# goalheart/ionic-mpnn

Hardware: AMD Instinct MI355X
Metric: molecule-graph pairs/sec (fwd), batch 4096 per MI355X (higher is better)
Workload: dtype f32 (bf16x9 emulation)

## Files before the change

ionic_mpnn_amd/csrc/api.hip:

```cpp
#include <cstring>
#include <vector>

#include <cstddef>

#include "common.h"
#include "encoder_layout.h"

namespace impnn {

char* error_buffer() {
  static thread_local char buf[512] = {0};
  return buf;
}

int fail(int code, const char* fmt, ...) {
  va_list ap;
  va_start(ap, fmt);
  vsnprintf(error_buffer(), 512, fmt, ap);
  va_end(ap);
  return code;
}

namespace {
struct Profiler {
// ... 313 lines not shown
                "indices or row offsets: split the batch", B, N, E, D);
  *bytes = encoder_fused_workspace_bytes(mode, n_ions, B, N, E, D, S, Vb, encoder_workgroups(n_ions, B, workgroups, N, E, mode));
  return IMPNN_OK;
}

int impnn_encoder_plan_layout(int32_t n_ions, int32_t B, int32_t N, int32_t E, int32_t D, int32_t K, int32_t S,
                              int32_t Vb, int32_t mode, int32_t workgroups, int64_t out[8]) {
  REQUIRE(out, "null pointer");
  size_t total = 0;
  if (int rc = impnn_encoder_workspace_bytes(n_ions, B, N, E, D, K, S, Vb, mode, workgroups, &total)) return rc;
  if (D != enc::kD)
    return fail(IMPNN_E_UNSUPPORTED, "encoder_plan_layout: atom_dim %d has no chunk plan (atom_dim 32 only)", D);
  const bool typed = mode >= 2;
  const int nwg = encoder_workgroups(n_ions, B, workgroups, N, E, mode);
  const enc::Ws w = enc::ws_layout(n_ions, B, N, E, S, Vb, nwg, typed, mode == 3);
  out[0] = w.nwg;
  out[1] = w.max_sub;
  out[2] = (int64_t)w.rows_off;
  out[3] = (int64_t)w.vr_off;
  out[4] = (int64_t)w.nsub_off;
  out[5] = (int64_t)w.desc_off;
  out[6] = typed ? enc::tecap_of(E) : 0;
  out[7] = enc::plan_vmin(n_ions, B, enc::vr_max_of(N, E, typed), w.nwg);
  return IMPNN_OK;
}

int impnn_encoder_plan_records(int32_t n_ions, int32_t B, int32_t N, int32_t E, int32_t D, int32_t K, int32_t S,
                               int32_t Vb, int32_t mode, int32_t workgroups, int64_t out[5]) {
  REQUIRE(out, "null pointer");
  size_t total = 0;
  if (int rc = impnn_encoder_workspace_bytes(n_ions, B, N, E, D, K, S, Vb, mode, workgroups, &total)) return rc;
  if (D != enc::kD)
    return fail(IMPNN_E_UNSUPPORTED, "encoder_plan_records: atom_dim %d has no chunk plan (atom_dim 32 only)", D);
  if (mode < 2)
    return fail(IMPNN_E_UNSUPPORTED, "encoder_plan_records: mode %d has pull-form records (typed modes only)", mode);
  const int nwg = encoder_workgroups(n_ions, B, workgroups, N, E, mode);
  const enc::Ws w = enc::ws_layout(n_ions, B, N, E, S, Vb, nwg, true, mode == 3);
  out[0] = (int64_t)w.rec_off;
  out[1] = w.rec_bytes;
  out[2] = enc::kTRecGrp;
  out[3] = enc::trec_runs_off(Vb, enc::tecap_of(E));
  out[4] = enc::kTRecNrun;
  return IMPNN_OK;
}

static int encoder_common(const char* fn, int32_t n_ions, const int32_t* const* atom_ids,
// ... 1632 lines not shown
```

ionic_mpnn_amd/csrc/common.h:

```cpp
#pragma once

#include <hip/hip_runtime.h>

#include <cstdarg>
#include <cstdint>
#include <cstdio>

#include "../../include/impnn.h"

namespace impnn {

char* error_buffer();
int fail(int code, const char* fmt, ...);

inline hipStream_t as_stream(impnn_stream_t s) { return reinterpret_cast<hipStream_t>(s); }

inline int check_launch(const char* what) {
  hipError_t e = hipGetLastError();
  if (e != hipSuccess) return fail(IMPNN_E_LAUNCH, "%s: %s", what, hipGetErrorString(e));
  return IMPNN_OK;
}

inline bool aligned16(const void* p) { return (reinterpret_cast<uintptr_t>(p) & 15u) == 0; }

// ... 422 lines not shown

void* debug_stamp_buffer(size_t* bytes);

struct EncoderArgs {
  int n_ions;
  const int32_t* atom_ids[2];
  const int32_t* bond_ids[2];
  const int32_t* conn[2];
  const float* weights[2];
  const void* prepared[2];
  int mode;
  int phases;
  int nwg;
  float* pooled[2];
  const float* atom_table;
  const float* bond_table;
  int Va, Vb, B, N, E, D, K, S;
  float ln_eps;
  void* workspace;
  size_t workspace_bytes;
};
bool encoder_fused_supported(int mode, int N, int E, int D, int K, int S, int Vb);
int encoder_workgroups(int n_ions, int B, int requested, int N, int E, int mode);
size_t encoder_fused_workspace_bytes(int mode, int n_ions, int B, int N, int E, int D, int S, int Vb, int nwg);
int launch_encoder_fused(const EncoderArgs& a, hipStream_t s);
int launch_encoder_phase(const EncoderArgs& a, hipStream_t s, bool plan_phase);
size_t encoder_prepared_bytes(int mode, int D, int S, int Vb);
int launch_encoder_prepare(const float* weights, const float* bond_table, int D, int K, int S, int Vb, int mode,
                           void* prepared, hipStream_t s);
size_t encoder_prepared_bytes_atoms(int mode, int D, int S, int Va, int Vb);
int launch_encoder_prepare_atoms(const float* weights, const float* bond_table, const float* atom_table, int Va, int D,
                                 int K, int S, int Vb, int mode, void* prepared, hipStream_t s);
size_t encoder_prepared_bytes_gates(int mode, int D, int S, int Va, int Vb);
int launch_encoder_prepare_gates(const float* weights, const float* bond_table, const float* atom_table, int Va, int D,
                                 int K, int S, int Vb, int mode, void* prepared, hipStream_t s);
int ensure_lds_limit(const void* kern, int slot);
int device_compute_units();
inline int gu_wide_tile_rows(int64_t rows) { return rows < 8192 ? 16 : 64; }
bool encoder_wide_supported(int N, int E, int D, int K, int S, int Vb);
size_t encoder_wide_workspace_bytes(int n_ions, int B, int N, int E, int D, int S, int Vb, bool x3);
bool encoder_wide_batch_covered(int n_ions, int B, int N, int E, int D, int Vb);
size_t encoder_wide_prepared_bytes(int D, int S, int Vb, bool x3);
int launch_encoder_wide_prepare(const float* weights, const float* bond_table, int D, int K, int S, int Vb, bool x3,
                                void* prepared, hipStream_t s);
int launch_encoder_wide(const EncoderArgs& a, hipStream_t s);

// ... 2 lines not shown
```

ionic_mpnn_amd/csrc/encoder_fused.hip:

```cpp
#include <atomic>
#include <cstdlib>

#include "encoder_device.h"
#include "encoder_layout.h"

namespace impnn {
namespace enc {

namespace {

struct H8 {
  half8 hi, lo;
};
__device__ __forceinline__ H8 split8(const float* v) {
  typedef __fp16 h2_t __attribute__((ext_vector_type(2)));
  union U {
    h2_t h;
    unsigned u;
  };
  union {
    half8 v8;
    unsigned u[4];
  } hi, lo;
#pragma unroll
// ... 452 lines not shown
  if (e != hipSuccess) return fail(IMPNN_E_LAUNCH, "encoder: cannot raise LDS limit: %s", hipGetErrorString(e));
  done[slot].fetch_or(bit, std::memory_order_release);
  return IMPNN_OK;
}

int encoder_workgroups(int n_ions, int B, int requested, int N, int E, int mode) {
  int cus = device_compute_units();
  int want = requested;
  if (want <= 0) {
    static const int env_want = [] {
      const char* e = getenv("IMPNN_ENCODER_WORKGROUPS");
      return e ? atoi(e) : 0;
    }();
    want = env_want;
  }
  if (want > 0) cus = want < 16 ? 16 : (want > cus ? cus : want);
  int f = 1;
  while ((int64_t)2 * n_ions * B / ((int64_t)cus * f) + 64 > enc::kShareCap ||
         enc::ws_layout(n_ions, B, N, E, 1, 1, cus * f, mode >= 2, mode == 3).max_sub > enc::kMaxHops)
    ++f;
  return cus * f;
}

size_t encoder_fused_workspace_bytes(int mode, int n_ions, int B, int N, int E, int D, int S, int Vb, int nwg) {
  if (D != enc::kD) return encoder_wide_workspace_bytes(n_ions, B, N, E, D, S, Vb, mode == 3);
  return enc::ws_layout(n_ions, B, N, E, S, Vb, nwg, mode >= 2, mode == 3).total;
}

size_t encoder_prepared_bytes(int mode, int D, int S, int Vb) {
  if (D != enc::kD) return encoder_wide_prepared_bytes(D, S, Vb, mode == 3);
  if (mode >= 2) return encoder_typed_prepared_bytes(S, Vb, mode == 3);
  return (size_t)(S > 0 ? S : 1) * enc::kImgSlot * sizeof(float);
}

int launch_encoder_prepare(const float* weights, const float* bond_table, int D, int K, int S, int Vb, int mode,
                           void* prepared, hipStream_t s) {
  if (S <= 0) return IMPNN_OK;
  if (D != enc::kD) return launch_encoder_wide_prepare(weights, bond_table, D, K, S, Vb, mode == 3, prepared, s);
  if (mode >= 2) return launch_encoder_typed_prepare(weights, bond_table, K, S, Vb, mode == 3, prepared, s);
  enc::ImageParams ip{};
  ip.weights = weights;
  ip.img = static_cast<float*>(prepared);
  ip.K = K;
  ip.mode = mode == 1 ? 1 : 0;
  ip.step_floats = impnn_encoder_step_floats(D, K);
  return enc::launch_weight_image(ip, S, s);
// ... 51 lines not shown
    ep.pooled[g] = a.pooled[g];
    if (plan_phase || typed) continue;
    if (a.prepared[g]) {
      if (!aligned16(a.prepared[g])) return fail(IMPNN_E_BADARG, "encoder_fused: prepared weights must be 16B aligned");
      ep.img[g] = static_cast<const float*>(a.prepared[g]);
    } else {
      float* img = reinterpret_cast<float*>(base + w.img_off) + (size_t)g * (a.S > 0 ? a.S : 1) * kImgSlot;
      if (int rc = launch_encoder_prepare(a.weights[g], a.bond_table, a.D, a.K, a.S, a.Vb, mode, img, s)) return rc;
      ep.img[g] = img;
    }
  }
  pp.rows = reinterpret_cast<int32_t*>(base + w.rows_off);
  pp.vr = reinterpret_cast<int32_t*>(base + w.vr_off);
  pp.partial = reinterpret_cast<int32_t*>(base + w.partial_off);
  pp.nsub = reinterpret_cast<int32_t*>(base + w.nsub_off);
  pp.desc = reinterpret_cast<int32_t*>(base + w.desc_off);
  pp.rec = reinterpret_cast<unsigned char*>(base + w.rec_off);
  pp.slist = reinterpret_cast<uint32_t*>(base + w.slist_off);
  pp.header = reinterpret_cast<PlanHeader*>(base);
  pp.typed = typed ? 1 : 0;
  pp.ecap = tecap_of(a.E);
  pp.vmin = plan_vmin(a.n_ions, a.B, vr_max_of(a.N, a.E, typed), w.nwg);
  pp.n_ions = a.n_ions; pp.B = a.B; pp.N = a.N; pp.E = a.E; pp.Va = a.Va; pp.Vb = a.Vb;
  {
    const int per_cu = typed ? 4 : 5;
    pp.grid_sub = w.max_sub < per_cu ? w.max_sub : per_cu;
  }
  pp.nwg = w.nwg;
  pp.max_sub = w.max_sub;
  pp.nblk = w.nblk;
  pp.stamps = nullptr;
  {
    size_t sb = 0;
    void* sp = debug_stamp_buffer(&sb);
    if (sp && sb >= ((size_t)w.nwg * 32 + 16) * sizeof(unsigned long long))
      pp.stamps = static_cast<unsigned long long*>(sp) + (size_t)w.nwg * 32;
  }
  if (plan_phase) return launch_plan(pp, s);
  if (typed) return launch_encoder_typed_run(a, w, s);

  ep.atom_table = a.atom_table;
  ep.bond_table = a.bond_table;
  ep.nsub = pp.nsub; ep.desc = pp.desc; ep.rec = pp.rec; ep.max_sub = w.max_sub;
  ep.header = pp.header;
  ep.n_ions = a.n_ions; ep.B = a.B; ep.N = a.N; ep.K = a.K; ep.S = a.S;
  ep.Va = a.Va; ep.Vb = a.Vb; ep.ln_eps = a.ln_eps;
  ep.stamps = nullptr;
  {
    size_t sb = 0;
    void* sp = debug_stamp_buffer(&sb);
// ... 20 lines not shown
```

ionic_mpnn_amd/csrc/encoder_layout.h:

```cpp
#pragma once

#include "common.h"

namespace impnn {
namespace enc {

typedef float f32x4 __attribute__((ext_vector_type(4)));
typedef _Float16 half8 __attribute__((ext_vector_type(8)));

constexpr float kSW = 256.0f;
constexpr float kSX = 16.0f;
constexpr float kAcc = kSW * kSX;

constexpr int kD = 32;
constexpr int kKMax = 8;
constexpr int kRCap = 256;
constexpr int kECap = 1024;
constexpr int kHS = 36;
constexpr int kMsgRS = 36;
constexpr int kUpdRS = 68;
constexpr int kThreads = 1024;
constexpr int kWaves = kThreads / 64;
constexpr int kTbCapFloats = 2048;

// ... 87 lines not shown
  const size_t n = (size_t)Vb * ((size_t)Va + 1) * kD;
  return n * sizeof(float) <= kM0CapBytes ? n : 0;
}

constexpr int32_t kG0Magic = 0x67307467;
constexpr int kG0Row = 2 * kD;
struct G0Header {
  int32_t magic, Va, Vb, S;
};
constexpr int kG0HeaderFloatOff = 4;
static_assert(sizeof(M0Header) == 4 * kG0HeaderFloatOff && kTUpdLds + 8 <= kTUpdSlot && kXUpdLds + 8 <= kXUpdSlot,
              "both headers fit the slot's tail");
inline size_t g0_table_floats(int S, int Va, int Vb) {
  return m0_table_floats(S, Va, Vb) ? ((size_t)Va + 1) * kG0Row : 0;
}

constexpr int kShareCap = kECap;
inline int plan_vmin(int n_ions, int B, int vrmax, int nwg) {
  const int64_t span = 2 * (int64_t)n_ions * B * vrmax / (nwg > 0 ? nwg : 1) + vrmax;
  const int64_t v = (span + kShareCap - 2) / (kShareCap - 1);
  return (int)(v < 1 ? 1 : (v > kRCap ? kRCap : v));
}
constexpr int kMaxHops = 128;

constexpr int kPB = 16;

struct Ws {
  size_t img_off, rows_off, vr_off, partial_off, share_off, nsub_off, desc_off, rec_off, slist_off, total;
  int nwg;
  int max_sub;
  int nblk;
  int rec_bytes;
};

inline size_t align_up(size_t x, size_t a) { return (x + a - 1) / a * a; }

__host__ __device__ constexpr int tvr_of_edges(int edges, int ecap) { return (edges * kRCap + ecap - 1) / ecap; }

inline int vr_max_of(int N, int E, bool typed = false) {
  int v = typed ? (E > 4 * kTECapBig ? kRCap + 1 : tvr_of_edges(E, tecap_of(E))) : (E + 3) / 4;
  int m = N > v ? N : v;
  m = m < 1 ? 1 : m;
  return typed && m > kRCap ? kRCap : m;
}

struct PlanHeader {
// ... 138 lines not shown
```

ionic_mpnn_amd/csrc/encoder_plan.hip:

```cpp
#include "encoder_layout.h"

namespace impnn {
namespace enc {

namespace {

__global__ __launch_bounds__(64 * kPB) void plan_stats_kernel(PlanParams p) {
  __shared__ int vsum[kPB], vbad[kPB];
  __builtin_amdgcn_s_setprio(3);
  const int lane = threadIdx.x & 63, wv = threadIdx.x >> 6;
  const int g = blockIdx.x / p.nblk, blk = blockIdx.x - g * p.nblk;
  const int b = blk * kPB + wv;
  const bool have = b < p.B;
  const int64_t item = (int64_t)g * p.B + (have ? b : 0);
  int my_vr = 0, my_bad = 0;
  if (have) {
  const int32_t* ids = p.atom_ids[g] + (int64_t)b * p.N;
  const int32_t* cn = p.conn[g] + (int64_t)b * p.E * 2;
  const int32_t* bd = p.bond_ids[g] + (int64_t)b * p.E;
  int rmax = 0, cnt = 0;
  const int id_first = lane < p.N ? ids[lane] : 0;
  int emax = 0;
  for (int e0 = 0; e0 < p.E; e0 += 256) {
    int2 st[4];
    int bid[4];
#pragma unroll
    for (int u = 0; u < 4; ++u) {
      const int e = e0 + 64 * u + lane;
      st[u] = make_int2(0, 0);
      bid[u] = -1;
      if (e < p.E) {
        st[u] = *reinterpret_cast<const int2*>(cn + 2 * e);
        bid[u] = bd[e];
      }
    }
#pragma unroll
    for (int u = 0; u < 4; ++u) {
      const bool ok = edge_valid(st[u].x, st[u].y, bid[u], p.N, p.Vb);
      if (ok) {
        const int m = st[u].x > st[u].y ? st[u].x : st[u].y;
        emax = emax > m ? emax : m;
      }
      cnt += __builtin_popcountll(__ballot(ok));
    }
  }
  {
    const unsigned long long hit = __ballot(id_first > 0);
    if (hit) rmax = 64 - __builtin_clzll(hit);
  }
  for (int n0 = 64; n0 < p.N; n0 += 64) {
    const int n = n0 + lane;
    const unsigned long long hit = __ballot(n < p.N && ids[n] > 0);
    if (hit) rmax = n0 + 64 - __builtin_clzll(hit);
  }
  if (cnt > 0) {
    bool alive = true;
// ... 3 lines not shown
      const bool one = alive && ((emax >> bit) & 1);
      if (__ballot(one)) {
        res |= 1 << bit;
        alive = one;
      }
    }
    rmax = rmax > res + 1 ? rmax : res + 1;
  }
  {
    int vr = p.typed ? tvr_of_edges(cnt < 0x100000 ? cnt : 0x100000, p.ecap) : (cnt + 3) >> 2;
    vr = vr > rmax ? vr : rmax;
    my_vr = vr < p.vmin ? p.vmin : vr;
    if (my_vr > kRCap) {
      my_vr = kRCap;
      my_bad = 1;
    }
    if (lane == 0) {
      p.rows[item] = rmax;
      p.vr[item] = my_vr;
    }
  }
  }
  if (lane == 0) {
    vsum[wv] = my_vr;
    vbad[wv] = my_bad;
  }
  lds_barrier();
  if (threadIdx.x == 0) {
    int t = 0, bad = 0;
#pragma unroll
    for (int i = 0; i < kPB; ++i) {
      t += vsum[i];
      bad |= vbad[i];
    }
    p.partial[(int64_t)g * p.nblk + blk] = t | (bad ? kPlanBadBit : 0);
    if (blockIdx.x == 0) {
      PlanHeader h;
      h.magic = kPlanMagic; h.kind = p.typed; h.n_ions = p.n_ions; h.B = p.B; h.N = p.N; h.E = p.E;
      h.nwg = p.nwg; h.max_sub = p.max_sub;
      h.overflow = 0;
      *p.header = h;
    }
  }
}


__global__ void weight_image_kernel(ImageParams p) {
  {
// ... 366 lines not shown
    int e = mb + 1;
    for (int c0 = mb + 1; c0 <= nsh; c0 += 64) {
      const int cidx = c0 + lane;
      const bool ok = cidx <= nsh && T.shst[cidx <= nsh ? cidx : nsh] <= lim;
      const unsigned long long okb = __ballot(ok);
      if (okb == 0) break;
      e = c0 + 63 - __builtin_clzll(okb);
      if (okb != ~0ull) break;
    }
    if (lane == 0) T.cb[hop] = mb;
    ++hop;
    mb = e;
  }
  if (lane == 0) {
    T.cb[hop] = nsh;
    T.chunk_s[0] = first;
    T.chunk_s[1] = hop;
    T.chunk_s[2] = g;
    if (slot_i == 0) p.nsub[j] = hop;
  }
}


__global__ __launch_bounds__(kRCap, 5) void plan_chunks_kernel(PlanParams p) {
  __shared__ int32_t moloff[kRCap + 2], molrows[kRCap], cnt[kRCap], place[kRCap], cursor[kRCap], rowptr[kRCap + 2];
  __shared__ int32_t bins[48], tilemax[16], scratch[8];
  __shared__ uint16_t atomof[kRCap];
  __shared__ uint32_t ent2[kECap + 1];
  __shared__ ShareTab T;
  __builtin_amdgcn_s_setprio(3);
  CSTAMP(0);
  const int j = blockIdx.x / p.grid_sub, slot_i = blockIdx.x - j * p.grid_sub;
  const int tid = threadIdx.x, lane = tid & 63, wave = tid >> 6;
  if (wave == 0) resolve_chain(p, j, slot_i, lane, T);
  lds_barrier();
  CSTAMP(1);
  const int first_mol = T.chunk_s[0], nhop = T.chunk_s[1], g = T.chunk_s[2];
  for (int sl = slot_i; sl < nhop; sl += p.grid_sub) {
  const int mb_local = T.cb[sl], M = T.cb[sl + 1] - mb_local, m0 = first_mol + mb_local;
  const int R = T.shst[mb_local + M] - T.shst[mb_local];
  const int idx = j * p.max_sub + sl;
  if (tid == 0) reinterpret_cast<int4*>(p.desc)[idx] = make_int4(m0, M, 0, R | (g << 16));
  const int N = p.N, E = p.E;
  const int32_t* ids_g = p.atom_ids[g];
  const int32_t* conn_g = p.conn[g];
  const int32_t* bond_g = p.bond_ids[g];
  const int32_t* rows_g = p.rows + (int64_t)g * p.B;
// ... 146 lines not shown
  {
    const int total = rowptr[kRCap];
    for (int i = tid; i < total; i += kRCap) {
      int lo = 0, hi = kRCap - 1;
      while (lo < hi) {
        const int mid = (lo + hi + 1) >> 1;
        if (rowptr[mid] <= i) lo = mid; else hi = mid - 1;
      }
      const int b0 = rowptr[lo], b1 = rowptr[lo + 1];
      const uint32_t v = ent2[i];
      int rank = 0;
      for (int jx = b0; jx < b1; ++jx) rank += ent2[jx] < v;
      const uint32_t srow = v & 0xffu, bid = (v >> 8) & 0xffu;
      const uint32_t aid = atomof[srow] < kEntMaxAtom ? atomof[srow] : kEntMaxAtom;
      r_ent[b0 + rank] = ((aid * (kHS / 4)) << 20) | ((srow * (kHS / 4)) << 8) | bid;
    }
  }
  CSTAMP(15);
  lds_barrier();
  }
}

constexpr int kTick = 16;
#ifndef IMPNN_T_RUNLPT
#define IMPNN_T_RUNLPT 1
#endif
constexpr bool kRunLpt = IMPNN_T_RUNLPT != 0;
static_assert(tgrp_cap(kTVbMax, kTECapBig) < 512, "group indices travel as 9 bits");
__device__ __forceinline__ int tgb_pack(int full_base, int full_groups, int rem_base) {
  return full_base | (full_groups << 9) | (rem_base << 18);
}
__device__ __forceinline__ int tgb_group(int w, int jg) {
  const int nfg = (w >> 9) & 511;
  return jg < nfg ? (w & 511) + jg : (w >> 18) + jg - nfg;
}
__global__ __launch_bounds__(kRCap, 4) void plan_chunks_typed_kernel(PlanParams p) {
  __shared__ int32_t moloff[kRCap + 2], molrows[kRCap], cnt[kRCap + 64], place[kRCap];
  __shared__ int32_t idl[kRCap];
  __shared__ __attribute__((aligned(16))) int32_t dbins[kRCap], dstart[kRCap], dcur[kRCap];
  __shared__ __attribute__((aligned(16))) int32_t thist[kTVbMax + 64], tgb[kTVbMax], tcur[kTVbMax + 64];
  __shared__ __attribute__((aligned(16))) int32_t jdp[kRCap + 4];
  __shared__ int32_t misc[4];
  __shared__ __attribute__((aligned(16))) uint16_t tick[kRCap * kTick];
  __shared__ uint2 elist[kTECapBig];
  extern __shared__ uint4 grp[];
  __shared__ ShareTab T;
  __builtin_amdgcn_s_setprio(3);
  CSTAMP(0);
  const int j = blockIdx.x / p.grid_sub, slot_i = blockIdx.x - j * p.grid_sub;
  const int tid = threadIdx.x, lane = tid & 63, wave = tid >> 6;
  if (wave == ((blockIdx.x >> 8) & 3)) resolve_chain(p, j, slot_i, lane, T);
  lds_barrier();
  CSTAMP(1);
  const int first_mol = T.chunk_s[0], nhop = T.chunk_s[1], g = T.chunk_s[2];
  const int N = p.N, E = p.E;
  const float rE = 1.0f / (float)E;
  for (int sl = slot_i; sl < nhop; sl += p.grid_sub) {
  const int mb_local = T.cb[sl], M = T.cb[sl + 1] - mb_local, m0 = first_mol + mb_local;
  const int base = T.shst[mb_local];
  const int R = T.shst[mb_local + M] - base;
  const int idx = j * p.max_sub + sl;
  const int32_t* ids_g = p.atom_ids[g];
  const int32_t* conn_g = p.conn[g];
  const int32_t* bond_g = p.bond_ids[g];
  const int32_t* rows_g = p.rows + (int64_t)g * p.B;
  unsigned char* rec = p.rec + (size_t)idx * kTRecBytes;
  uint32_t* r_slist = p.slist + (size_t)idx * p.ecap;
  uint16_t* r_rowdeg = reinterpret_cast<uint16_t*>(rec + kTRecRowdeg);
  unsigned char* r_tilemax = rec + kTRecTilemax;
  uint16_t* r_moloff = reinterpret_cast<uint16_t*>(rec + kTRecMoloff);
  uint16_t* r_molrows = reinterpret_cast<uint16_t*>(rec + kTRecMolrows);
  uint16_t* r_poolrow = reinterpret_cast<uint16_t*>(rec + kTRecPoolrow);
  int32_t* r_rowatom = reinterpret_cast<int32_t*>(rec + kTRecRowatom);
  uint16_t* r_jd = reinterpret_cast<uint16_t*>(rec + kTRecJdptr);
  uint16_t* r_cw = reinterpret_cast<uint16_t*>(rec + kTRecCounts);

  const int n_slots = M * E;
  constexpr int kSC = 6;
  int sbid[kSC];
  int2 sst[kSC];
  const int32_t* conn_c = conn_g + (int64_t)m0 * E * 2;
  const int32_t* bond_c = bond_g + (int64_t)m0 * E;
#pragma unroll
  for (int k = 0; k < kSC; ++k) {
    const int slot = tid + k * kRCap;
    sbid[k] = -1; sst[k] = make_int2(0, 0);
    if (slot < n_slots) {
      sst[k] = *reinterpret_cast<const int2*>(conn_c + 2 * (int64_t)slot);
      sbid[k] = bond_c[slot];
    }
  }
  constexpr int kIC = 3;
  const int n_ids = M * N;
  const float rN = 1.0f / (float)N;
  const int32_t* ids_c = ids_g + (int64_t)m0 * N;
  int sid[kIC];
#pragma unroll
  for (int k = 0; k < kIC; ++k) {
    const int slot = tid + k * kRCap;
    sid[k] = slot < n_ids ? ids_c[slot] : 0;
  }
  for (int m = tid; m <= M; m += kRCap) {
    const int off = T.shst[mb_local + m] - base;
    moloff[m] = off;
    r_moloff[m] = (uint16_t)off;
    if (m < M) {
      const int rr = rows_g[m0 + m];
      molrows[m] = rr;
      r_molrows[m] = (uint16_t)rr;
    }
  }
  cnt[tid] = 0;
  dbins[tid] = 0;
  dcur[tid] = 0;
  thist[tid] = 0;
  tcur[tid] = 0;
  idl[tid] = -1;
  if (tid == 0) misc[1] = 0;
  {
    const uint4 ones = make_uint4(~0u, ~0u, ~0u, ~0u);
    reinterpret_cast<uint4*>(tick)[2 * tid] = ones;
    reinterpret_cast<uint4*>(tick)[2 * tid + 1] = ones;
  }
  lds_barrier();
  CSTAMP(2);

  auto put_id = [&](int slot, int id) {
    const int m = fast_div(slot, N, rN), n = slot - m * N;
    if (slot < n_ids && n < molrows[m]) idl[moloff[m] + n] = id;
  };
  {
    const int dq = fast_div(kRCap, N, rN), dr = kRCap - dq * N;
    int cm = fast_div(tid, N, rN), cn = tid - cm * N;
    int mr[kIC], mo[kIC], nn[kIC];
#pragma unroll
    for (int k = 0; k < kIC; ++k) {
      const int mm = tid + k * kRCap < n_ids ? cm : 0;
      mr[k] = tid + k * kRCap < n_ids ? molrows[mm] : 0;
      mo[k] = moloff[mm];
// ... 22 lines not shown
      int row[3], srw[3], tk[3], es[3];
#pragma unroll
      for (int k = 0; k < 3; ++k) {
        const bool ok = (okm >> (k0 + k)) & 1u;
        const int m = cm;
        es[k] = ce;
        ce += dr; cm += dq;
        if (ce >= E) { ce -= E; ++cm; }
        const int mo = moloff[m < M ? m : 0];
        row[k] = mo + (ok ? sst[k0 + k].y : 0);
        srw[k] = mo + (ok ? sst[k0 + k].x : 0);
      }
#pragma unroll
      for (int k = 0; k < 3; ++k) {
        const bool ok = (okm >> (k0 + k)) & 1u;
        tk[k] = atomicAdd(&cnt[ok ? row[k] : kRCap + lane], 1);
        atomicAdd(&thist[ok ? sbid[k0 + k] : kTVbMax + lane], 1);
      }
#pragma unroll
      for (int k = 0; k < 3; ++k) {
        const bool ok = (okm >> (k0 + k)) & 1u;
        if (ok && tk[k] < kTick) tick[row[k] * kTick + tk[k]] = (uint16_t)es[k];
        if (ok) {
          if (pos < kTECapBig)
            elist[pos] = make_uint2((uint32_t)row[k] | ((uint32_t)srw[k] << 8) | ((uint32_t)sbid[k0 + k] << 16), (uint32_t)es[k]);
          ++pos;
        }
      }
    }
  }
  for (int s0 = kSC * kRCap; s0 < n_slots; s0 += kRCap) {
    const int slot = s0 + tid;
    int2 st = make_int2(0, 0);
    int bid = -1;
    if (slot < n_slots) {
      st = *reinterpret_cast<const int2*>(conn_c + 2 * (int64_t)slot);
      bid = bond_c[slot];
    }
    const bool ok = edge_valid(st.x, st.y, bid, N, p.Vb);
    const int m = fast_div(slot, E, rE), e = slot - m * E;
    const int mo = moloff[m < M ? m : 0];
    const int row = mo + (ok ? st.y : 0);
    int tk = kTick;
    if (ok) {
      tk = atomicAdd(&cnt[row], 1);
      atomicAdd(&thist[bid], 1);
    }
    const unsigned long long okb = __ballot(ok);
    int pos0 = 0;
    if (okb != 0ull) {
      if (lane == (int)__builtin_ctzll(okb)) pos0 = atomicAdd(&misc[1], (int)__builtin_popcountll(okb));
      pos0 = __builtin_amdgcn_readlane(pos0, (int)__builtin_ctzll(okb));
    }
    if (tk < kTick) tick[row * kTick + tk] = (uint16_t)e;
    const int pos = pos0 + (int)__builtin_popcountll(okb & ((1ull << lane) - 1));
    if (ok && pos < kTECapBig)
      elist[pos] = make_uint2((uint32_t)row | ((uint32_t)(mo + st.x) << 8) | ((uint32_t)bid << 16), (uint32_t)e);
  }
  lds_barrier();
  CSTAMP(3);

  const int my_deg = cnt[tid];
  const int dcl = my_deg > 255 ? 255 : my_deg;
  if (tid < R) {
    if (my_deg > 255) p.header->overflow = 1;
    atomicAdd(&dbins[255 - dcl], 1);
  }
  lds_barrier();
  CSTAMP(4);

  if (wave == 0) {
    const int4 h = reinterpret_cast<const int4*>(dbins)[lane];
    const int s4 = h.x + h.y + h.z + h.w;
    const int ex = wave_incl_scan(s4) - s4;
    reinterpret_cast<int4*>(dstart)[lane] = make_int4(ex, ex + h.x, ex + h.x + h.y, ex + h.x + h.y + h.z);
    __builtin_amdgcn_s_waitcnt(0xc07f);
    const int4 s = reinterpret_cast<const int4*>(dstart)[63 - lane];
    const int t4 = s.x + s.y + s.z + s.w;
    const int incl = wave_incl_scan(t4);
    const int jx = incl - t4;
    reinterpret_cast<int4*>(jdp)[lane] = make_int4(jx, jx + s.w, jx + s.w + s.z, jx + s.w + s.z + s.y);
    if (lane == 63) { jdp[kRCap] = incl; jdp[kRCap + 1] = incl; }
  } else if (wave == 1) {
    const int4 n = reinterpret_cast<const int4*>(thist)[lane];
    const int4 ng = make_int4((n.x + 3) >> 2, (n.y + 3) >> 2, (n.z + 3) >> 2, (n.w + 3) >> 2);
    const int s4 = ng.x + ng.y + ng.z + ng.w;
    const int incl = wave_incl_scan(s4);
    const int ex = incl - s4;
    const int ngrp_all = __builtin_amdgcn_readlane(incl, 63);
    int gmax = (ngrp_all + kTRunTarget - 1) / kTRunTarget;
    gmax = gmax < 2 ? 2 : gmax;
    const float rgm = 1.0f / (float)gmax;
    uint16_t* runs = reinterpret_cast<uint16_t*>(rec + trec_runs_off(p.Vb, p.ecap));
    if (kRunLpt) {
      const int ngv[4] = {ng.x, ng.y, ng.z, ng.w};
      int nf[4], rem[4];
#pragma unroll
      for (int i = 0; i < 4; ++i) {
        nf[i] = fast_div(ngv[i], gmax, rgm);
        rem[i] = ngv[i] - nf[i] * gmax;
      }
      const int f4 = nf[0] + nf[1] + nf[2] + nf[3];
      const int fincl = wave_incl_scan(f4);
      static_assert(kTRunTarget <= 64, "one lane per full run");
      const int nfull = __builtin_amdgcn_readlane(fincl, 63);
// ... 56 lines not shown
  }
  lds_barrier();
  CSTAMP(5);

  int pos = tid;
  if (tid < R) pos = dstart[255 - dcl] + atomicAdd(&dcur[255 - dcl], 1);
  place[tid] = pos;
  {
    const int my_id = idl[tid];
    r_rowatom[pos] = my_id;
    r_poolrow[tid] = (uint16_t)(pos | (my_id > 0 ? 0x8000 : 0));
    r_rowdeg[pos] = (uint16_t)my_deg;
    if ((pos & 15) == 0) r_tilemax[pos >> 4] = (unsigned char)dcl;
    r_jd[tid] = (uint16_t)jdp[tid];
    if (tid < 2) r_jd[kRCap + tid] = (uint16_t)jdp[kRCap];
    if (pos == 0) {
      r_cw[0] = (uint16_t)misc[0];
      r_cw[1] = (uint16_t)jdp[kRCap];
      r_cw[2] = (uint16_t)dcl;
    }
    if (tid == 0)
      reinterpret_cast<int4*>(p.desc)[idx] = make_int4(m0, M, jdp[kRCap] < p.ecap ? jdp[kRCap] : p.ecap, R | (g << 16));
  }
  {
    const int n_t = thist[tid];
    const int ng = (n_t + 3) >> 2, gb = tgb[tid];
    const uint32_t dump = (uint32_t)tmsg_key(p.ecap) * 0x10001u;
    for (int jg = 0; jg < ng; ++jg) {
      const int c = n_t - 4 * jg;
      grp[tgb_group(gb, jg)] = make_uint4((uint32_t)tid | ((uint32_t)(c < 4 ? c : 4) << 8) |
                                              (kRunLpt ? 0u : (uint32_t)(ng - jg) << 24), 0u, dump, dump);
    }
  }
  lds_barrier();
  CSTAMP(6);

  {
    auto below = [](uint4 a, uint32_t ue) {
      return (int)(((a.x & 0xffffu) < ue) + ((a.x >> 16) < ue) + ((a.y & 0xffffu) < ue) + ((a.y >> 16) < ue) +
                   ((a.z & 0xffffu) < ue) + ((a.z >> 16) < ue) + ((a.w & 0xffffu) < ue) + ((a.w >> 16) < ue));
    };
    const int nval = misc[1] < kTECapBig ? misc[1] : kTECapBig;
    for (int i0 = 0; i0 < nval; i0 += 2 * kRCap) {
      bool ok[2];
      uint2 en[2];
      int row[2], srow[2], deg[2], ix[2], gb[2], rank[2];
      uint4 ta[2], tb[2];
#pragma unroll
      for (int k = 0; k < 2; ++k) {
        const int i = i0 + k * kRCap + tid;
        ok[k] = i < nval;
        en[k] = elist[ok[k] ? i : 0];
      }
#pragma unroll
      for (int k = 0; k < 2; ++k) {
        const int rt = (int)(en[k].x & 0xffu), bid = (int)(en[k].x >> 16);
        deg[k] = cnt[rt];
        ta[k] = reinterpret_cast<const uint4*>(tick)[2 * rt];
        tb[k] = reinterpret_cast<const uint4*>(tick)[2 * rt + 1];
        row[k] = place[rt];
        srow[k] = place[(en[k].x >> 8) & 0xffu];
        gb[k] = tgb[bid];
        ix[k] = atomicAdd(&tcur[ok[k] ? bid : kTVbMax + lane], 1);
      }
#pragma unroll
      for (int k = 0; k < 2; ++k) {
        rank[k] = below(ta[k], en[k].y) + below(tb[k], en[k].y);
        if (deg[k] > kTick) {
          const int rt = (int)(en[k].x & 0xffu);
          int lo = 0, hi = M - 1;
          while (lo < hi) {
            const int mid = (lo + hi + 1) >> 1;
            if (moloff[mid] <= rt) lo = mid; else hi = mid - 1;
          }
          const int t = rt - moloff[lo];
          const int32_t* cm = conn_c + 2 * (int64_t)lo * E;
          const int32_t* bm = bond_c + (int64_t)lo * E;
          rank[k] = 0;
          for (int e2 = 0; e2 < (int)en[k].y; ++e2) {
            const int2 s2 = *reinterpret_cast<const int2*>(cm + 2 * e2);
            rank[k] += (s2.y == t && edge_valid(s2.x, s2.y, bm[e2], N, p.Vb)) ? 1 : 0;
          }
        }
        rank[k] = jdp[rank[k] < 256 ? rank[k] : 255];
      }
#pragma unroll
      for (int k = 0; k < 2; ++k) {
        if (ok[k]) {
          unsigned char* ge = reinterpret_cast<unsigned char*>(&grp[tgb_group(gb[k], ix[k] >> 2)]);
          ge[4 + (ix[k] & 3)] = (unsigned char)srow[k];
          reinterpret_cast<uint16_t*>(ge + 8)[ix[k] & 3] = (uint16_t)tmsg_key(rank[k] + row[k]);
          if (rank[k] + row[k] < p.ecap)
            r_slist[rank[k] + row[k]] = tsrc_word((int)(en[k].x >> 16), idl[(en[k].x >> 8) & 0xffu]);
        }
      }
    }
  }
  lds_barrier();
  CSTAMP(9);

  {
    const int ngrp = misc[0];
    uint4* r_grp = reinterpret_cast<uint4*>(rec + kTRecGrp);
    for (int i = tid; i < ngrp; i += kRCap) r_grp[i] = grp[i];
  }
  CSTAMP(15);
  lds_barrier();
  }
}
#undef CSTAMP

}

int launch_weight_image(const ImageParams& ip, int S, hipStream_t s) {
  if (S <= 0) return IMPNN_OK;
  weight_image_kernel<<<dim3(16, S), 256, 0, s>>>(ip);
  return check_launch("weight_image");
}

int launch_typed_image(const TImageParams& ip, hipStream_t s) {
  const int S = ip.S > 0 ? ip.S : 1;
  float* canon = ip.prepared + (size_t)S * (ip.x3 ? kXUpdSlot : kTUpdSlot) + (size_t)S * ip.Vb * kTMatFloats;
  for (int st = 0; st < ip.S; ++st) {
    if (int rc = launch_bond_type_matrices(ip.bond_table, ip.weights + (int64_t)st * ip.step_floats, canon, ip.Vb, ip.K,
                                           kD, s))
      return rc;
    typed_image_kernel<<<(ip.Vb * kTMatFloats + kTUpdSlot + 255) / 256 < 256 ? (ip.Vb * kTMatFloats + kTUpdSlot + 255) / 256 : 256,
                         256, 0, s>>>(ip, st);
    if (int rc = check_launch("typed_image")) return rc;
  }
  return IMPNN_OK;
}

int launch_plan(const PlanParams& pp, hipStream_t s) {
  plan_stats_kernel<<<pp.n_ions * pp.nblk, 64 * kPB, 0, s>>>(pp);
  if (int rc = check_launch("plan_stats")) return rc;
  if ((int64_t)2 * pp.n_ions * pp.B / pp.nwg + 64 > kShareCap)
    return fail(IMPNN_E_UNSUPPORTED, "encoder plan: batch of %d molecules per ion is too large", pp.B);
  if (pp.max_sub > kMaxHops)
    return fail(IMPNN_E_UNSUPPORTED, "encoder plan: %d chunk slots per workgroup", pp.max_sub);
  if (pp.typed)
    plan_chunks_typed_kernel<<<pp.nwg * pp.grid_sub, kRCap, sizeof(uint4) * tgrp_cap(pp.Vb, pp.ecap), s>>>(pp);
  else
    plan_chunks_kernel<<<pp.nwg * pp.grid_sub, kRCap, 0, s>>>(pp);
  return check_launch("plan_chunks");
}

}
}
```

Baseline: 42.81 million.

## Shrink typed plan-builder LDS to run more builder blocks per CU

Restructures the typed chunk-planning kernel's shared memory into a templated struct that aliases the share table, ticket array and group table in one arena and narrows several arrays to 16-bit. This lets the small-edge-cap variant run 8 blocks per CU instead of 4, and the grid sub-count now scales with device CU count divided by workgroups. Later hops recompute molecule offsets with a wave scan instead of keeping share tables resident. The stats kernel also prefetches the first edge tile per molecule. The aliasing adds extra barriers and depends on the tickets being dead before the group table is written.

```diff
diff --git a/ionic_mpnn_amd/csrc/api.hip b/ionic_mpnn_amd/csrc/api.hip
--- a/ionic_mpnn_amd/csrc/api.hip
+++ b/ionic_mpnn_amd/csrc/api.hip
@@ -359,6 +359,28 @@
   out[5] = (int64_t)w.desc_off;
   out[6] = typed ? enc::tecap_of(E) : 0;
   out[7] = enc::plan_vmin(n_ions, B, enc::vr_max_of(N, E, typed), w.nwg);
+  return IMPNN_OK;
+}
+
+int impnn_encoder_plan_grid(int32_t n_ions, int32_t B, int32_t N, int32_t E, int32_t D, int32_t K, int32_t S, int32_t Vb,
+                            int32_t mode, int32_t workgroups, int32_t cus, int64_t out[5]) {
+  REQUIRE(out, "null pointer");
+  REQUIRE(cus >= 0, "cus must be >= 0 (0: the current device)");
+  int64_t lay[8];
+  if (int rc = impnn_encoder_plan_layout(n_ions, B, N, E, D, K, S, Vb, mode, workgroups, lay)) return rc;
+  const int per_cu = enc::plan_builders_per_cu(mode >= 2, E);
+  const int n_cus = cus > 0 ? cus : device_compute_units();
+  out[0] = plan_grid_sub((int)lay[1], per_cu, n_cus, (int)lay[0]);
+  out[1] = per_cu;
+  out[2] = n_cus;
+  out[3] = lay[1];
+  out[4] = lay[0];
+  return IMPNN_OK;
+}
+
+int impnn_debug_set_plan_builders(int32_t per_share) {
+  REQUIRE(per_share >= 0, "per_share must be >= 0 (0: default)");
+  debug_set_plan_builders_cap(per_share);
   return IMPNN_OK;
 }
 
diff --git a/ionic_mpnn_amd/csrc/common.h b/ionic_mpnn_amd/csrc/common.h
--- a/ionic_mpnn_amd/csrc/common.h
+++ b/ionic_mpnn_amd/csrc/common.h
@@ -468,6 +468,8 @@
 };
 bool encoder_fused_supported(int mode, int N, int E, int D, int K, int S, int Vb);
 int encoder_workgroups(int n_ions, int B, int requested, int N, int E, int mode);
+int plan_grid_sub(int max_sub, int builders_per_cu, int cus, int nwg);
+void debug_set_plan_builders_cap(int cap);
 size_t encoder_fused_workspace_bytes(int mode, int n_ions, int B, int N, int E, int D, int S, int Vb, int nwg);
 int launch_encoder_fused(const EncoderArgs& a, hipStream_t s);
 int launch_encoder_phase(const EncoderArgs& a, hipStream_t s, bool plan_phase);
diff --git a/ionic_mpnn_amd/csrc/encoder_fused.hip b/ionic_mpnn_amd/csrc/encoder_fused.hip
--- a/ionic_mpnn_amd/csrc/encoder_fused.hip
+++ b/ionic_mpnn_amd/csrc/encoder_fused.hip
@@ -498,6 +498,18 @@
   return cus * f;
 }
 
+int plan_grid_sub(int max_sub, int builders_per_cu, int cus, int nwg) {
+  int64_t g = (int64_t)builders_per_cu * cus / (nwg > 0 ? nwg : 1);
+  g = g < max_sub ? g : max_sub;
+  return (int)(g < 1 ? 1 : g);
+}
+
+#ifndef IMPNN_DIAG_PLAN_BUILDERS_CAP
+#define IMPNN_DIAG_PLAN_BUILDERS_CAP 0
+#endif
+static std::atomic<int> g_plan_builders_cap{IMPNN_DIAG_PLAN_BUILDERS_CAP};
+void debug_set_plan_builders_cap(int cap) { g_plan_builders_cap.store(cap > 0 ? cap : 0, std::memory_order_relaxed); }
+
 size_t encoder_fused_workspace_bytes(int mode, int n_ions, int B, int N, int E, int D, int S, int Vb, int nwg) {
   if (D != enc::kD) return encoder_wide_workspace_bytes(n_ions, B, N, E, D, S, Vb, mode == 3);
   return enc::ws_layout(n_ions, B, N, E, S, Vb, nwg, mode >= 2, mode == 3).total;
@@ -595,10 +607,8 @@
   pp.ecap = tecap_of(a.E);
   pp.vmin = plan_vmin(a.n_ions, a.B, vr_max_of(a.N, a.E, typed), w.nwg);
   pp.n_ions = a.n_ions; pp.B = a.B; pp.N = a.N; pp.E = a.E; pp.Va = a.Va; pp.Vb = a.Vb;
-  {
-    const int per_cu = typed ? 4 : 5;
-    pp.grid_sub = w.max_sub < per_cu ? w.max_sub : per_cu;
-  }
+  pp.grid_sub = plan_grid_sub(w.max_sub, plan_builders_per_cu(typed, a.E), device_compute_units(), w.nwg);
+  if (const int cap = g_plan_builders_cap.load(std::memory_order_relaxed)) pp.grid_sub = pp.grid_sub < cap ? pp.grid_sub : cap;
   pp.nwg = w.nwg;
   pp.max_sub = w.max_sub;
   pp.nblk = w.nblk;
diff --git a/ionic_mpnn_amd/csrc/encoder_layout.h b/ionic_mpnn_amd/csrc/encoder_layout.h
--- a/ionic_mpnn_amd/csrc/encoder_layout.h
+++ b/ionic_mpnn_amd/csrc/encoder_layout.h
@@ -133,6 +133,14 @@
   return (int)(v < 1 ? 1 : (v > kRCap ? kRCap : v));
 }
 constexpr int kMaxHops = 128;
+
+#ifndef IMPNN_DIAG_T_BUILDERS_PER_CU
+#define IMPNN_DIAG_T_BUILDERS_PER_CU 8
+#endif
+constexpr int kPullBuildersPerCu = 5, kTBuildersPerCu = IMPNN_DIAG_T_BUILDERS_PER_CU, kTBuildersPerCuBig = 4;
+inline int plan_builders_per_cu(bool typed, int E) {
+  return !typed ? kPullBuildersPerCu : (tecap_of(E) == kTECap ? kTBuildersPerCu : kTBuildersPerCuBig);
+}
 
 constexpr int kPB = 16;
 
diff --git a/ionic_mpnn_amd/csrc/encoder_plan.hip b/ionic_mpnn_amd/csrc/encoder_plan.hip
--- a/ionic_mpnn_amd/csrc/encoder_plan.hip
+++ b/ionic_mpnn_amd/csrc/encoder_plan.hip
@@ -5,12 +5,41 @@
 
 namespace {
 
-__global__ __launch_bounds__(64 * kPB) void plan_stats_kernel(PlanParams p) {
+#ifndef IMPNN_PLAN_MOL_PER_WAVE
+#define IMPNN_PLAN_MOL_PER_WAVE 1
+#endif
+constexpr int kMolPerWave = IMPNN_PLAN_MOL_PER_WAVE;
+static_assert(kMolPerWave == 1 || kMolPerWave == 2 || kMolPerWave == 4, "a block of kPB molecules in whole waves");
+constexpr int kStatsThreads = 64 * kPB / kMolPerWave;
+__global__ __launch_bounds__(kStatsThreads) void plan_stats_kernel(PlanParams p) {
   __shared__ int vsum[kPB], vbad[kPB];
   __builtin_amdgcn_s_setprio(3);
   const int lane = threadIdx.x & 63, wv = threadIdx.x >> 6;
   const int g = blockIdx.x / p.nblk, blk = blockIdx.x - g * p.nblk;
-  const int b = blk * kPB + wv;
+  int2 st0[kMolPerWave][4];
+  int bid0[kMolPerWave][4], id0[kMolPerWave];
+#pragma unroll
+  for (int q = 0; q < kMolPerWave; ++q) {
+    const int b = blk * kPB + wv * kMolPerWave + q;
+    const bool have = b < p.B;
+    const int32_t* ids = p.atom_ids[g] + (int64_t)(have ? b : 0) * p.N;
+    const int32_t* cn = p.conn[g] + (int64_t)(have ? b : 0) * p.E * 2;
+    const int32_t* bd = p.bond_ids[g] + (int64_t)(have ? b : 0) * p.E;
+    id0[q] = have && lane < p.N ? ids[lane] : 0;
+#pragma unroll
+    for (int u = 0; u < 4; ++u) {
+      const int e = 64 * u + lane;
+      st0[q][u] = make_int2(0, 0);
+      bid0[q][u] = -1;
+      if (have && e < p.E) {
+        st0[q][u] = *reinterpret_cast<const int2*>(cn + 2 * e);
+        bid0[q][u] = bd[e];
+      }
+    }
+  }
+#pragma unroll
+  for (int q = 0; q < kMolPerWave; ++q) {
+  const int b = blk * kPB + wv * kMolPerWave + q;
   const bool have = b < p.B;
   const int64_t item = (int64_t)g * p.B + (have ? b : 0);
   int my_vr = 0, my_bad = 0;
@@ -19,7 +48,7 @@
   const int32_t* cn = p.conn[g] + (int64_t)b * p.E * 2;
   const int32_t* bd = p.bond_ids[g] + (int64_t)b * p.E;
   int rmax = 0, cnt = 0;
-  const int id_first = lane < p.N ? ids[lane] : 0;
+  const int id_first = id0[q];
   int emax = 0;
   for (int e0 = 0; e0 < p.E; e0 += 256) {
     int2 st[4];
@@ -27,11 +56,15 @@
 #pragma unroll
     for (int u = 0; u < 4; ++u) {
       const int e = e0 + 64 * u + lane;
-      st[u] = make_int2(0, 0);
-      bid[u] = -1;
-      if (e < p.E) {
-        st[u] = *reinterpret_cast<const int2*>(cn + 2 * e);
-        bid[u] = bd[e];
+      st[u] = st0[q][u];
+      bid[u] = bid0[q][u];
+      if (e0 > 0) {
+        st[u] = make_int2(0, 0);
+        bid[u] = -1;
+        if (e < p.E) {
+          st[u] = *reinterpret_cast<const int2*>(cn + 2 * e);
+          bid[u] = bd[e];
+        }
       }
     }
 #pragma unroll
@@ -81,8 +114,9 @@
   }
   }
   if (lane == 0) {
-    vsum[wv] = my_vr;
-    vbad[wv] = my_bad;
+    vsum[wv * kMolPerWave + q] = my_vr;
+    vbad[wv * kMolPerWave + q] = my_bad;
+  }
   }
   lds_barrier();
   if (threadIdx.x == 0) {
@@ -495,7 +529,7 @@
 }
 
 
-__global__ __launch_bounds__(kRCap, 5) void plan_chunks_kernel(PlanParams p) {
+__global__ __launch_bounds__(kRCap, kPullBuildersPerCu) void plan_chunks_kernel(PlanParams p) {
   __shared__ int32_t moloff[kRCap + 2], molrows[kRCap], cnt[kRCap], place[kRCap], cursor[kRCap], rowptr[kRCap + 2];
   __shared__ int32_t bins[48], tilemax[16], scratch[8];
   __shared__ uint16_t atomof[kRCap];
@@ -688,6 +722,13 @@
 }
 
 constexpr int kTick = 16;
+__device__ __forceinline__ int turn_local(int v) {
+  asm volatile("" : "+v"(v));
+  return v;
+}
+#ifndef IMPNN_DIAG_PLAN_LDS_PAD
+#define IMPNN_DIAG_PLAN_LDS_PAD 0
+#endif
 #ifndef IMPNN_T_RUNLPT
 #define IMPNN_T_RUNLPT 1
 #endif
@@ -700,31 +741,73 @@
   const int nfg = (w >> 9) & 511;
   return jg < nfg ? (w & 511) + jg : (w >> 18) + jg - nfg;
 }
-__global__ __launch_bounds__(kRCap, 4) void plan_chunks_typed_kernel(PlanParams p) {
-  __shared__ int32_t moloff[kRCap + 2], molrows[kRCap], cnt[kRCap + 64], place[kRCap];
-  __shared__ int32_t idl[kRCap];
-  __shared__ __attribute__((aligned(16))) int32_t dbins[kRCap], dstart[kRCap], dcur[kRCap];
-  __shared__ __attribute__((aligned(16))) int32_t thist[kTVbMax + 64], tgb[kTVbMax], tcur[kTVbMax + 64];
-  __shared__ __attribute__((aligned(16))) int32_t jdp[kRCap + 4];
-  __shared__ int32_t misc[4];
-  __shared__ __attribute__((aligned(16))) uint16_t tick[kRCap * kTick];
-  __shared__ uint2 elist[kTECapBig];
-  extern __shared__ uint4 grp[];
-  __shared__ ShareTab T;
+template <int kEC>
+struct TypedLds {
+  static constexpr bool kGrpInArena = kEC == kTECap;
+  __attribute__((aligned(16))) unsigned char arena[kRCap * kTick * sizeof(uint16_t)];
+  int32_t cnt[kRCap + 64];
+  int32_t idl[kRCap];
+  __attribute__((aligned(16))) int32_t dbins[kRCap];
+  __attribute__((aligned(16))) int32_t thist[kTVbMax + 64];
+  __attribute__((aligned(16))) int32_t tgb[kTVbMax];
+  uint2 elist[kEC];
+  __attribute__((aligned(8))) uint16_t dstart[kRCap];
+  __attribute__((aligned(8))) uint16_t jdp[kRCap + 4];
+  uint16_t moloff[kRCap + 2], molrows[kRCap];
+  uint16_t cbk[kMaxHops + 2];
+  int32_t misc[4];
+};
+static_assert(sizeof(ShareTab) <= sizeof(TypedLds<kTECap>::arena), "the share tables lie where the tickets will");
+static_assert(sizeof(uint4) * tgrp_cap(kTVbMax, kTECap) <= sizeof(TypedLds<kTECap>::arena), "the group table lies where the tickets did");
+static_assert(sizeof(TypedLds<kTECap>) * kTBuildersPerCu <= 160 * 1024, "plan_chunks_typed: more LDS than an eighth of a CU's");
+static_assert((sizeof(TypedLds<kTECapBig>) + sizeof(uint4) * tgrp_cap(kTVbMax, kTECapBig)) * kTBuildersPerCuBig <= 160 * 1024,
+              "plan_chunks_typed, records of kTECapBig edges: more LDS than a quarter of a CU's");
+
+template <int kEC>
+__global__ __launch_bounds__(kRCap, kEC == kTECap ? kTBuildersPerCu : kTBuildersPerCuBig) void plan_chunks_typed_kernel(PlanParams p) {
+  constexpr bool kGrpInArena = TypedLds<kEC>::kGrpInArena;
+  __shared__ TypedLds<kEC> L;
+  extern __shared__ uint4 grp_dyn[];
+  auto& cnt = L.cnt; auto& idl = L.idl; auto& dbins = L.dbins; auto& dcur = L.dbins; auto& thist = L.thist;
+  auto& tcur = L.thist; auto& tgb = L.tgb; auto& elist = L.elist; auto& dstart = L.dstart; auto& jdp = L.jdp;
+  auto& moloff = L.moloff; auto& molrows = L.molrows; auto& place = L.molrows; auto& misc = L.misc;
+  ShareTab& T = *reinterpret_cast<ShareTab*>(L.arena);
+  uint16_t* const tick = reinterpret_cast<uint16_t*>(L.arena);
+  uint4* const grp = kGrpInArena ? reinterpret_cast<uint4*>(L.arena) : grp_dyn;
   __builtin_amdgcn_s_setprio(3);
   CSTAMP(0);
   const int j = blockIdx.x / p.grid_sub, slot_i = blockIdx.x - j * p.grid_sub;
   const int tid = threadIdx.x, lane = tid & 63, wave = tid >> 6;
-  if (wave == ((blockIdx.x >> 8) & 3)) resolve_chain(p, j, slot_i, lane, T);
-  lds_barrier();
-  CSTAMP(1);
-  const int first_mol = T.chunk_s[0], nhop = T.chunk_s[1], g = T.chunk_s[2];
+  const int rwave = (blockIdx.x >> 8) & 3;
   const int N = p.N, E = p.E;
   const float rE = 1.0f / (float)E;
+  if (wave == rwave) resolve_chain(p, j, slot_i, lane, T);
+  lds_barrier();
+  CSTAMP(1);
+  const int first_mol = __builtin_amdgcn_readfirstlane(T.chunk_s[0]), nhop = __builtin_amdgcn_readfirstlane(T.chunk_s[1]), g = __builtin_amdgcn_readfirstlane(T.chunk_s[2]);
+  if (slot_i + p.grid_sub < nhop && tid <= nhop) L.cbk[tid] = (uint16_t)T.cb[tid];
   for (int sl = slot_i; sl < nhop; sl += p.grid_sub) {
-  const int mb_local = T.cb[sl], M = T.cb[sl + 1] - mb_local, m0 = first_mol + mb_local;
-  const int base = T.shst[mb_local];
-  const int R = T.shst[mb_local + M] - base;
+  const int tid = turn_local(threadIdx.x), lane = tid & 63, wave = tid >> 6;
+  int mb_local, M, R, my_off;
+  if (sl == slot_i) {
+    mb_local = __builtin_amdgcn_readfirstlane(T.cb[sl]);
+    M = __builtin_amdgcn_readfirstlane(T.cb[sl + 1]) - mb_local;
+    const int base = __builtin_amdgcn_readfirstlane(T.shst[mb_local]);
+    R = __builtin_amdgcn_readfirstlane(T.shst[mb_local + M]) - base;
+    my_off = T.shst[mb_local + (tid < M ? tid : M)] - base;
+  } else {
+    mb_local = __builtin_amdgcn_readfirstlane((int)L.cbk[sl]);
+    M = __builtin_amdgcn_readfirstlane((int)L.cbk[sl + 1]) - mb_local;
+    const int v = tid < M ? p.vr[(int64_t)g * p.B + first_mol + mb_local + tid] : 0;
+    const int incl = wave_incl_scan(v);
+    if (lane == 63) misc[wave] = incl;
+    lds_barrier();
+    const int w0 = misc[0], w1 = misc[1], w2 = misc[2], w3 = misc[3];
+    R = __builtin_amdgcn_readfirstlane(w0 + w1 + w2 + w3);
+    my_off = incl - v + (wave > 0 ? w0 : 0) + (wave > 1 ? w1 : 0) + (wave > 2 ? w2 : 0);
+    if (tid >= M) my_off = R;
+  }
+  const int m0 = first_mol + mb_local;
   const int idx = j * p.max_sub + sl;
   const int32_t* ids_g = p.atom_ids[g];
   const int32_t* conn_g = p.conn[g];
@@ -766,21 +849,24 @@
     const int slot = tid + k * kRCap;
     sid[k] = slot < n_ids ? ids_c[slot] : 0;
   }
-  for (int m = tid; m <= M; m += kRCap) {
-    const int off = T.shst[mb_local + m] - base;
-    moloff[m] = off;
-    r_moloff[m] = (uint16_t)off;
-    if (m < M) {
-      const int rr = rows_g[m0 + m];
-      molrows[m] = rr;
-      r_molrows[m] = (uint16_t)rr;
-    }
+  const int my_rows = tid < M ? rows_g[m0 + tid] : 0;
+  lds_barrier();
+  CSTAMP(7);
+  if (tid <= M) {
+    moloff[tid] = (uint16_t)my_off;
+    r_moloff[tid] = (uint16_t)my_off;
+  }
+  if (tid == 0 && M == kRCap) {
+    moloff[kRCap] = (uint16_t)R;
+    r_moloff[kRCap] = (uint16_t)R;
+  }
+  if (tid < M) {
+    molrows[tid] = (uint16_t)my_rows;
+    r_molrows[tid] = (uint16_t)my_rows;
   }
   cnt[tid] = 0;
   dbins[tid] = 0;
-  dcur[tid] = 0;
   thist[tid] = 0;
-  tcur[tid] = 0;
   idl[tid] = -1;
   if (tid == 0) misc[1] = 0;
   {
@@ -849,7 +935,7 @@
         const bool ok = (okm >> (k0 + k)) & 1u;
         if (ok && tk[k] < kTick) tick[row[k] * kTick + tk[k]] = (uint16_t)es[k];
         if (ok) {
-          if (pos < kTECapBig)
+          if (pos < kEC)
             elist[pos] = make_uint2((uint32_t)row[k] | ((uint32_t)srw[k] << 8) | ((uint32_t)sbid[k0 + k] << 16), (uint32_t)es[k]);
           ++pos;
         }
@@ -881,7 +967,7 @@
     }
     if (tk < kTick) tick[row * kTick + tk] = (uint16_t)e;
     const int pos = pos0 + (int)__builtin_popcountll(okb & ((1ull << lane) - 1));
-    if (ok && pos < kTECapBig)
+    if (ok && pos < kEC)
       elist[pos] = make_uint2((uint32_t)row | ((uint32_t)(mo + st.x) << 8) | ((uint32_t)bid << 16), (uint32_t)e);
   }
   lds_barrier();
@@ -898,16 +984,24 @@
 
   if (wave == 0) {
     const int4 h = reinterpret_cast<const int4*>(dbins)[lane];
+    {
+      const int z = turn_local(0);
+      reinterpret_cast<int4*>(dcur)[lane] = make_int4(z, z, z, z);
+    }
     const int s4 = h.x + h.y + h.z + h.w;
     const int ex = wave_incl_scan(s4) - s4;
-    reinterpret_cast<int4*>(dstart)[lane] = make_int4(ex, ex + h.x, ex + h.x + h.y, ex + h.x + h.y + h.z);
+    auto pack4 = [](int a, int b, int c, int d) {
+      return make_uint2((uint32_t)a | ((uint32_t)b << 16), (uint32_t)c | ((uint32_t)d << 16));
+    };
+    reinterpret_cast<uint2*>(dstart)[lane] = pack4(ex, ex + h.x, ex + h.x + h.y, ex + h.x + h.y + h.z);
     __builtin_amdgcn_s_waitcnt(0xc07f);
-    const int4 s = reinterpret_cast<const int4*>(dstart)[63 - lane];
+    const uint2 sp = reinterpret_cast<const uint2*>(dstart)[63 - lane];
+    const int4 s = make_int4((int)(sp.x & 0xffffu), (int)(sp.x >> 16), (int)(sp.y & 0xffffu), (int)(sp.y >> 16));
     const int t4 = s.x + s.y + s.z + s.w;
     const int incl = wave_incl_scan(t4);
     const int jx = incl - t4;
-    reinterpret_cast<int4*>(jdp)[lane] = make_int4(jx, jx + s.w, jx + s.w + s.z, jx + s.w + s.z + s.y);
-    if (lane == 63) { jdp[kRCap] = incl; jdp[kRCap + 1] = incl; }
+    reinterpret_cast<uint2*>(jdp)[lane] = pack4(jx, jx + s.w, jx + s.w + s.z, jx + s.w + s.z + s.y);
+    if (lane == 63) { jdp[kRCap] = (uint16_t)incl; jdp[kRCap + 1] = (uint16_t)incl; }
   } else if (wave == 1) {
     const int4 n = reinterpret_cast<const int4*>(thist)[lane];
     const int4 ng = make_int4((n.x + 3) >> 2, (n.y + 3) >> 2, (n.z + 3) >> 2, (n.w + 3) >> 2);
@@ -1010,8 +1104,9 @@
     if (tid == 0)
       reinterpret_cast<int4*>(p.desc)[idx] = make_int4(m0, M, jdp[kRCap] < p.ecap ? jdp[kRCap] : p.ecap, R | (g << 16));
   }
-  {
-    const int n_t = thist[tid];
+  const int n_t = thist[tid];
+  tcur[tid] = 0;
+  if (!kGrpInArena) {
     const int ng = (n_t + 3) >> 2, gb = tgb[tid];
     const uint32_t dump = (uint32_t)tmsg_key(p.ecap) * 0x10001u;
     for (int jg = 0; jg < ng; ++jg) {
@@ -1028,7 +1123,7 @@
       return (int)(((a.x & 0xffffu) < ue) + ((a.x >> 16) < ue) + ((a.y & 0xffffu) < ue) + ((a.y >> 16) < ue) +
                    ((a.z & 0xffffu) < ue) + ((a.z >> 16) < ue) + ((a.w & 0xffffu) < ue) + ((a.w >> 16) < ue));
     };
-    const int nval = misc[1] < kTECapBig ? misc[1] : kTECapBig;
+    const int nval = misc[1] < kEC ? misc[1] : kEC;
     for (int i0 = 0; i0 < nval; i0 += 2 * kRCap) {
       bool ok[2];
       uint2 en[2];
@@ -1072,6 +1167,22 @@
         }
         rank[k] = jdp[rank[k] < 256 ? rank[k] : 255];
       }
+      if (kGrpInArena) {
+        lds_barrier();
+        CSTAMP(8);
+        const int ng = (n_t + 3) >> 2, gbt = tgb[tid];
+        const uint16_t dump16 = (uint16_t)tmsg_key(p.ecap);
+        for (int jg = 0; jg < ng; ++jg) {
+          const int c = n_t - 4 * jg;
+          unsigned char* ge = reinterpret_cast<unsigned char*>(&grp[tgb_group(gbt, jg)]);
+          *reinterpret_cast<uint32_t*>(ge) = (uint32_t)tid | ((uint32_t)(c < 4 ? c : 4) << 8) |
+                                             (kRunLpt ? 0u : (uint32_t)(ng - jg) << 24);
+          for (int l = c; l < 4; ++l) {
+            ge[4 + l] = 0;
+            reinterpret_cast<uint16_t*>(ge + 8)[l] = dump16;
+          }
+        }
+      }
 #pragma unroll
       for (int k = 0; k < 2; ++k) {
         if (ok[k]) {
@@ -1093,6 +1204,7 @@
     for (int i = tid; i < ngrp; i += kRCap) r_grp[i] = grp[i];
   }
   CSTAMP(15);
+  if (sl + p.grid_sub >= nhop) break;
   lds_barrier();
   }
 }
@@ -1121,14 +1233,16 @@
 }
 
 int launch_plan(const PlanParams& pp, hipStream_t s) {
-  plan_stats_kernel<<<pp.n_ions * pp.nblk, 64 * kPB, 0, s>>>(pp);
+  plan_stats_kernel<<<pp.n_ions * pp.nblk, kStatsThreads, 0, s>>>(pp);
   if (int rc = check_launch("plan_stats")) return rc;
   if ((int64_t)2 * pp.n_ions * pp.B / pp.nwg + 64 > kShareCap)
     return fail(IMPNN_E_UNSUPPORTED, "encoder plan: batch of %d molecules per ion is too large", pp.B);
   if (pp.max_sub > kMaxHops)
     return fail(IMPNN_E_UNSUPPORTED, "encoder plan: %d chunk slots per workgroup", pp.max_sub);
-  if (pp.typed)
-    plan_chunks_typed_kernel<<<pp.nwg * pp.grid_sub, kRCap, sizeof(uint4) * tgrp_cap(pp.Vb, pp.ecap), s>>>(pp);
+  if (pp.typed && pp.ecap == kTECap)
+    plan_chunks_typed_kernel<kTECap><<<pp.nwg * pp.grid_sub, kRCap, IMPNN_DIAG_PLAN_LDS_PAD, s>>>(pp);
+  else if (pp.typed)
+    plan_chunks_typed_kernel<kTECapBig><<<pp.nwg * pp.grid_sub, kRCap, sizeof(uint4) * tgrp_cap(pp.Vb, pp.ecap), s>>>(pp);
   else
     plan_chunks_kernel<<<pp.nwg * pp.grid_sub, kRCap, 0, s>>>(pp);
   return check_launch("plan_chunks");
```

After: 39.85 million. -6.9%, worse.
